# ami-iit/jaxsim

Measured on AMD Instinct MI355X. Metric: env-steps/sec (whole node), iCub 23-DoF soft-contact, batch 1024/8192, higher is better.
Workload: dtype f32

## Files before the change

### include/jaxsim_amd.h

```cpp
#ifndef JAXSIM_AMD_H
#define JAXSIM_AMD_H

#include <stdint.h>

#ifdef __cplusplus
extern "C" {
#endif

#define JXS_OK 0
#define JXS_EINVAL (-1)
#define JXS_ENODEVICE (-2)
#define JXS_ENOMEM (-3)
#define JXS_ECOMM (-4)

#define JXS_F32 0
#define JXS_F64 1

#define JXS_REPR_INERTIAL 0
#define JXS_REPR_BODY 1
#define JXS_REPR_MIXED 2

#define JXS_INTEGRATOR_SEMI_IMPLICIT_EULER 0
#define JXS_INTEGRATOR_RUNGE_KUTTA4 1
#define JXS_INTEGRATOR_RUNGE_KUTTA4_FAST 2
// ... 6 lines not shown
  int32_t n_links;
  int32_t floating_base;
  int32_t dtype;
  const int32_t* parent;
  const int32_t* joint_type;
  const double* joint_axis;
  const double* lambda_H_pre;
  const double* suc_H_i;
  const double* link_mass;
  const double* link_com;
  const double* link_inertia;
  const double* friction_static;
  const double* friction_viscous;
  const double* position_limit_min;
  const double* position_limit_max;
  const double* position_limit_spring;
  const double* position_limit_damper;
  int32_t n_points;
  const int32_t* point_body;
  const double* point_position;
  const uint8_t* point_enabled;
  double time_step;
  double gravity;
  double K, D, mu, p, q;
  double terrain_height;
  double torque_max, omega_th, omega_max;
  int32_t enable_friction;
  double terrain_normal[3];
  int32_t integrator;
  int32_t contact_model;
  double regularization_delassus;
  double solver_tol;
  double rr_time_constant, rr_damping_coefficient, rr_d_min, rr_d_max, rr_width, rr_midpoint, rr_power;
  const double* terrain_grid;
  int32_t terrain_nx, terrain_ny;
  double terrain_origin[2];
  double terrain_spacing[2];
  double terrain_delta;
} jxs_model_desc;

typedef struct jxs_model jxs_model;

typedef struct jxs_layout {
  int32_t n_links, n_joints, n_points, n_rows;
  int32_t row_pos, row_quat, row_s, row_vlin, row_vang, row_sd, row_m;
  int32_t group;
  int32_t tile;
  int32_t dtype;
  int32_t row_mode;
} jxs_layout;

const char* jxs_last_error(void);
int jxs_device_count(int* count);
int jxs_set_device(int device);
int jxs_malloc(void** dptr, uint64_t bytes);
int jxs_free(void* dptr);
int jxs_memcpy_h2d(void* dst, const void* src, uint64_t bytes, void* stream);
int jxs_memcpy_d2h(void* dst, const void* src, uint64_t bytes, void* stream);
int jxs_memcpy_d2d(void* dst, const void* src, uint64_t bytes, void* stream);
int jxs_memset(void* dst, int value, uint64_t bytes, void* stream);
int jxs_stream_create(void** stream);
int jxs_stream_destroy(void* stream);
int jxs_stream_synchronize(void* stream);
int jxs_stream_wait_spin(void* stream);
int jxs_device_synchronize(void);
int jxs_event_create(void** event);
int jxs_event_destroy(void* event);
int jxs_event_record(void* event, void* stream);
int jxs_event_elapsed_ms(void* start, void* stop, float* ms);

int jxs_model_create(const jxs_model_desc* desc, jxs_model** out);
int jxs_model_destroy(jxs_model* model);
int jxs_model_layout(const jxs_model* model, jxs_layout* out);

enum { JXS_MODE_STEP = 0, JXS_MODE_STEP_RIGID = 6 };
int jxs_kernel_spec(const jxs_model_desc* desc, int mode, char* buf, int capacity);
int jxs_model_attach_specialized(jxs_model* model, int mode, const char* shared_object_path);
int jxs_model_specialized_modes(const jxs_model* model, unsigned* mask);


int jxs_step(jxs_model* model, const void* state_in, void* state_out, const void* tau,
             const void* link_forces, int force_repr, int N, void* stream);

int jxs_step_repeat(jxs_model* model, void* state, const void* tau, const void* link_forces,
                    int force_repr, int N, int n_launches, void* stream);

int jxs_step_repeat_timed(jxs_model* model, void* state, const void* tau, const void* link_forces,
                          int force_repr, int N, int n_launches, void* stream, double* seconds);

int jxs_rollout(jxs_model* model, void* state, const void* tau, const void* link_forces,
                int force_repr, int N, int n_steps, void* stream);

int jxs_rollout_controlled(jxs_model* model, void* state, const void* tau_seq, const void* link_forces,
                           int force_repr, int N, int n_steps, void* stream);

int jxs_rollout_recorded(jxs_model* model, void* state, const void* tau, int tau_per_step, const void* link_forces,
                         int force_repr, int N, int n_steps, void* out_states, void* stream);

int jxs_forward_dynamics_aba(jxs_model* model, const void* state, const void* joint_forces,
                             const void* link_forces, int force_repr, void* out_acc, int N,
                             void* stream);

int jxs_system_dynamics(jxs_model* model, const void* state, const void* joint_torques, const void* link_forces,
                        int force_repr, double baumgarte, void* out_xdot, void* out_link_contact_forces, int N,
                        void* stream);
int jxs_link_contact_forces(jxs_model* model, const void* state, const void* joint_torques, const void* link_forces,
                            int force_repr, void* out_link_contact_forces, void* out_mdot, int N, void* stream);

int jxs_inverse_dynamics(jxs_model* model, const void* state, const void* in_acc,
                         const void* link_forces, int force_repr, void* out_forces, int N,
                         void* stream);

int jxs_tile_from_env_major(const void* src, void* dst, int rows, int N, int tile, int dtype, void* stream);
int jxs_tile_to_env_major(const void* src, void* dst, int rows, int N, int tile, int dtype, void* stream);

int jxs_validate_state(jxs_model* model, const void* state, int N, int* counts3, void* stream);

int jxs_env_select(const uint8_t* mask, const void* a, const void* b, void* out, int rows, int N, int tile, int dtype,
                   void* stream);

int jxs_env_copy(const void* src, int src_N, int src_tile, const int32_t* src_idx, void* dst, int dst_N, int dst_tile,
                 const int32_t* dst_idx, int rows, int K, int dtype, void* stream);

enum { JXS_ENV_NONFINITE = 1, JXS_ENV_QUAT_NOT_UNIT = 2 };
int jxs_env_flags(jxs_model* model, const void* state, int N, uint8_t* out_flags, void* stream);

int jxs_env_randomize(jxs_model* model, const uint8_t* mask, void* state, int N, const void* bounds, uint64_t seed,
                      uint64_t draw, int64_t first_env, int velocity_representation, void* stream);

#define JXS_OBS_MAX_WIDTH 4096
enum {
  JXS_OBS_STATE_ROW = 0,
  JXS_OBS_SOURCE_ROW = 1,
  JXS_OBS_BASE_QUAT_UNIT = 2,
  JXS_OBS_BASE_ROTATION = 3,
  JXS_OBS_BASE_VELOCITY = 4,
  JXS_OBS_PROJECTED_GRAVITY = 5
};
typedef struct jxs_observation jxs_observation;
int jxs_observation_create(jxs_model* model, int D, const int32_t* slots , const double* offset,
                           const double* scale, const int32_t source_rows[4], jxs_observation** out);
int jxs_observation_destroy(jxs_observation* observation);
int jxs_env_observe(jxs_model* model, const jxs_observation* observation, const void* state,
                    const void* const sources[4], int N, int velocity_representation, void* out, int out_dtype,
                    int64_t out_ld, void* stream);

#define JXS_ACT_MAX_WIDTH 4096
enum { JXS_ACT_OFF = 0, JXS_ACT_TORQUE = 1, JXS_ACT_POSITION = 2, JXS_ACT_VELOCITY = 3 };
typedef struct jxs_action jxs_action;
int jxs_action_create(jxs_model* model, int A, const int32_t* joints ,
                      const double* params , jxs_action** out);
int jxs_action_destroy(jxs_action* action);
int jxs_env_act(jxs_model* model, const jxs_action* action, const void* state, const void* actions, int act_dtype,
                int64_t act_ld, const void* feed_forward, void* out_tau, int N, void* stream);

#define JXS_EVAL_MAX_SLOTS 1024
#define JXS_EVAL_MAX_TERMS 32
#define JXS_EVAL_MAX_CONDITIONS 32
#define JXS_DONE_TERMINATED 1
#define JXS_DONE_TRUNCATED 2
enum { JXS_EVAL_IDENTITY = 0, JXS_EVAL_ABS = 1, JXS_EVAL_SQUARE = 2, JXS_EVAL_EXCESS = 3 };
enum { JXS_EVAL_OUTER_IDENTITY = 0, JXS_EVAL_OUTER_EXP = 1 };
enum { JXS_EVAL_TERMINATED = 0, JXS_EVAL_TRUNCATED = 1 };
typedef struct jxs_evaluation_desc {
  int32_t D, K, C;
  const int32_t* slots;
  const int32_t* targets;
  const double* offset;
// ... 96 lines not shown
```

### jaxsim_amd/_lib.py

```python

from __future__ import annotations

import ctypes as C
import os
import pathlib

import numpy as np

_HERE = pathlib.Path(__file__).resolve().parent
LIB_PATH = _HERE / "csrc" / "libjaxsim_amd.so"

JXS_F32, JXS_F64 = 0, 1


class JaxsimAmdError(RuntimeError):
    pass


class ModelDesc(C.Structure):

    _fields_ = [
        ("n_links", C.c_int32),
        ("floating_base", C.c_int32),
        ("dtype", C.c_int32),
# ... 159 lines not shown
    d.regularization_delassus = float(getattr(cm, "regularization_delassus", 1e-6))
    d.solver_tol = float(getattr(cm, "solver_tol", 1e-3))
    return d, keep


def model_signature(model, dtype) -> tuple:
    kdp = model.kin_dyn_parameters
    cp, ap = model.contact_params, model.actuation_params
    return (
        id(kdp), np.dtype(dtype).str, model.time_step, model.gravity, model.floating_base(),
        cp.K, cp.D, cp.mu, getattr(cp, "p", 0.5), getattr(cp, "q", 0.5), model.terrain._height, tuple(getattr(model.terrain, "_normal", (0.0, 0.0, 1.0))),
        ap.torque_max, ap.omega_th, ap.omega_max, ap.enable_friction, int(model.integrator),
        type(model.contact_model).__name__, getattr(model.contact_model, "regularization_delassus", None),
        getattr(model.contact_model, "solver_tol", None),
        tuple(getattr(cp, k, None) for k in ("time_constant", "damping_coefficient", "d_min", "d_max", "width", "midpoint", "power")),
        (id(getattr(model.terrain, "_heights", None)), getattr(model.terrain, "_origin", None), getattr(model.terrain, "_spacing", None),
         getattr(model.terrain, "delta", None)) if getattr(model.terrain, "_heights", None) is not None else None,
    )


_lib = None


def _declare(lib):
    vp, cp_ = C.c_void_p, C.c_char_p
    lib.jxs_last_error.restype = cp_
    lib.jxs_last_error.argtypes = []
    sig = {
        "jxs_device_count": [C.POINTER(C.c_int)],
        "jxs_set_device": [C.c_int],
        "jxs_malloc": [C.POINTER(vp), C.c_uint64],
        "jxs_free": [vp],
        "jxs_memcpy_h2d": [vp, vp, C.c_uint64, vp],
        "jxs_memcpy_d2h": [vp, vp, C.c_uint64, vp],
        "jxs_memcpy_d2d": [vp, vp, C.c_uint64, vp],
        "jxs_memset": [vp, C.c_int, C.c_uint64, vp],
        "jxs_stream_create": [C.POINTER(vp)],
        "jxs_stream_destroy": [vp],
        "jxs_stream_synchronize": [vp],
        "jxs_stream_wait_spin": [vp],
        "jxs_device_synchronize": [],
        "jxs_event_create": [C.POINTER(vp)],
        "jxs_event_destroy": [vp],
        "jxs_event_record": [vp, vp],
        "jxs_event_elapsed_ms": [vp, vp, C.POINTER(C.c_float)],
        "jxs_model_create": [C.POINTER(ModelDesc), C.POINTER(vp)],
        "jxs_kernel_spec": [C.POINTER(ModelDesc), C.c_int, C.c_char_p, C.c_int],
        "jxs_model_attach_specialized": [vp, C.c_int, C.c_char_p],
        "jxs_model_specialized_modes": [vp, C.POINTER(C.c_uint)],
        "jxs_model_destroy": [vp],
        "jxs_model_layout": [vp, C.POINTER(Layout)],
        "jxs_step": [vp, vp, vp, vp, vp, C.c_int, C.c_int, vp],
        "jxs_step_gravity_compensated": [vp, vp, vp, vp, vp, C.c_int, C.c_int, vp],
        "jxs_rollout": [vp, vp, vp, vp, C.c_int, C.c_int, C.c_int, vp],
        "jxs_rollout_controlled": [vp, vp, vp, vp, C.c_int, C.c_int, C.c_int, vp],
        "jxs_rollout_recorded": [vp, vp, vp, C.c_int, vp, C.c_int, C.c_int, C.c_int, vp, vp],
        "jxs_forward_dynamics_aba": [vp, vp, vp, vp, C.c_int, vp, C.c_int, vp],
        "jxs_forward_dynamics_crb": [vp, vp, vp, vp, C.c_int, vp, C.c_int, vp],
        "jxs_inverse_dynamics": [vp, vp, vp, vp, C.c_int, vp, C.c_int, vp],
        "jxs_system_dynamics": [vp, vp, vp, vp, C.c_int, C.c_double, vp, vp, C.c_int, vp],
        "jxs_link_contact_forces": [vp, vp, vp, vp, C.c_int, vp, vp, C.c_int, vp],
        "jxs_gravity_torques": [vp, vp, vp, C.c_int, vp],
        "jxs_tile_from_env_major": [vp, vp, C.c_int, C.c_int, C.c_int, C.c_int, vp],
        "jxs_tile_to_env_major": [vp, vp, C.c_int, C.c_int, C.c_int, C.c_int, vp],
        "jxs_validate_state": [vp, vp, C.c_int, C.POINTER(C.c_int), vp],
        "jxs_env_select": [vp, vp, vp, vp, C.c_int, C.c_int, C.c_int, C.c_int, vp],
        "jxs_env_copy": [vp, C.c_int, C.c_int, vp, vp, C.c_int, C.c_int, vp, C.c_int, C.c_int, C.c_int, vp],
        "jxs_env_flags": [vp, vp, C.c_int, vp, vp],
        "jxs_env_randomize": [vp, vp, vp, C.c_int, vp, C.c_uint64, C.c_uint64, C.c_int64, C.c_int, vp],
        "jxs_observation_create": [vp, C.c_int, C.POINTER(C.c_int32), C.POINTER(C.c_double), C.POINTER(C.c_double), C.POINTER(C.c_int32), C.POINTER(vp)],
        "jxs_observation_destroy": [vp],
        "jxs_env_observe": [vp, vp, vp, C.POINTER(vp), C.c_int, C.c_int, vp, C.c_int, C.c_int64, vp],
        "jxs_action_create": [vp, C.c_int, C.POINTER(C.c_int32), C.POINTER(C.c_double), C.POINTER(vp)],
        "jxs_action_destroy": [vp],
        "jxs_env_act": [vp, vp, vp, vp, C.c_int, C.c_int64, vp, vp, C.c_int, vp],
        "jxs_evaluation_create": [vp, C.POINTER(EvaluationDesc), C.POINTER(vp)],
        "jxs_evaluation_destroy": [vp],
        "jxs_env_evaluate": [vp, vp, vp, C.POINTER(vp), C.c_int, C.c_int, vp, C.c_int, vp, vp, vp, C.c_int, C.c_int64, vp, C.c_int, vp],
        "jxs_contact_sensors_create": [vp, C.c_int, C.POINTER(C.c_int32), C.c_int, C.POINTER(C.c_int32), C.POINTER(C.c_double), C.POINTER(vp)],
        "jxs_contact_sensors_destroy": [vp],
        "jxs_env_contacts": [vp, vp, vp, vp, C.c_int, C.c_double, vp, vp, vp, vp],
        "jxs_step_repeat": [vp, vp, vp, vp, C.c_int, C.c_int, C.c_int, vp],
        "jxs_step_repeat_timed": [vp, vp, vp, vp, C.c_int, C.c_int, C.c_int, vp, C.POINTER(C.c_double)],
        "jxs_refresh_kinematics": [vp, vp, vp, vp, C.c_int, vp],
        "jxs_mass_matrix": [vp, vp, vp, C.c_int, vp],
        "jxs_centroidal": [vp, vp, vp, vp, C.c_int, vp],
        "jxs_coriolis": [vp, vp, vp, vp, C.c_int, vp],
        "jxs_frames_create": [vp, C.c_int, C.POINTER(C.c_int32), C.POINTER(C.c_double), C.POINTER(vp)],
        "jxs_frames_destroy": [vp],
        "jxs_frame_kinematics": [vp, vp, vp, C.c_int, C.c_int, vp, vp, C.c_int, vp],
        "jxs_solver_fault_counts": [vp, C.POINTER(C.c_int), C.c_int, vp],
        "jxs_debug_reload_env": [],
        "jxs_jacobian_full": [vp, vp, vp, vp, C.c_int, vp],
        "jxs_mass_matrix_inverse": [vp, vp, vp, C.c_int, vp],
        "jxs_comm_unique_id": [C.c_char * 128],
        "jxs_comm_version": [C.POINTER(C.c_int)],
        "jxs_device_pci_bus_id": [C.c_char_p, C.c_int],
        "jxs_comm_init": [C.POINTER(vp), C.c_char * 128, C.c_int, C.c_int],
        "jxs_comm_destroy": [vp],
        "jxs_allgather": [vp, vp, vp, C.c_uint64, C.c_int, vp],
    }
    for name, args in sig.items():
        fn = getattr(lib, name)
        fn.restype = C.c_int
        fn.argtypes = args
    return sig


EXPORTED_SYMBOLS = None


def load(path: os.PathLike | None = None):
    global _lib, EXPORTED_SYMBOLS
    if _lib is not None and path is None:
        return _lib
    override = os.environ.get("JAXSIM_AMD_LIB")
    p = pathlib.Path(path) if path is not None else (pathlib.Path(override) if override else LIB_PATH)
    if not p.exists():
        raise JaxsimAmdError(
            f"HIP extension not built: {p} is missing. Run `python -c 'import __graft_entry__ as g; g.build()'` "
            "(or jaxsim_amd/csrc/build.sh). There is no CPU fallback."
        )
    try:
        lib = C.CDLL(str(p))
    except OSError as e:
        raise JaxsimAmdError(f"cannot load {p}: {e}") from e
    EXPORTED_SYMBOLS = tuple(_declare(lib).keys()) + ("jxs_last_error",)
    if path is None:
        _lib = lib
    return lib


def check(rc: int, what: str = "") -> None:
    if rc != 0:
        msg = load().jxs_last_error()
        raise JaxsimAmdError(f"{what} failed ({rc}): {msg.decode() if msg else ''}")
```

### jaxsim_amd/csrc/jxs_api.hip

```cpp
#include <cstdint>
#include <dlfcn.h>
#include <hip/hip_runtime.h>

#include <algorithm>
#include <atomic>
#include <chrono>
#include <rccl/rccl.h>

#include <cstdlib>
#include <cstring>
#include <map>
#include <memory>
#include <mutex>
#include <string>
#include <type_traits>

#include "../../include/jaxsim_amd.h"
#include "jxs_env_act.h"
#include "jxs_env_contact.h"
#include "jxs_env_evaluate.h"
#include "jxs_env_observe.h"
#include "jxs_env_ops.h"
#include "jxs_env_random.h"
#include "jxs_params.h"
// ... 887 lines not shown

namespace {

int refuse(const char* who, const std::string& what) { return fail(JXS_EINVAL, std::string(who) + ": " + what); }

bool repr_ok(int r) { return r == JXS_REPR_INERTIAL || r == JXS_REPR_BODY || r == JXS_REPR_MIXED; }

struct EnvTile {
  int tile = 0, tile_shift = 0;
};
int env_tile(const char* who, int G, int rows, EnvTile& t) {
  t.tile = G > 0 ? 64 / G : 0, t.tile_shift = 0;
  while ((1 << t.tile_shift) < t.tile) ++t.tile_shift;
  if (t.tile <= 0 || (1 << t.tile_shift) != t.tile || t.tile > 64) return refuse(who, "the model's tile does not divide the wave");
  if (jxs_env::tile_words(rows, t.tile) >= (1LL << 30)) return refuse(who, "rows * tile must be below 2^30");
  return JXS_OK;
}

template <int WB, typename F>
void with_access(int access, F&& f) {
  if (access == 16) f(std::integral_constant<int, 16>{});
  else if (access == 8) f(std::integral_constant<int, 8>{});
  else if constexpr (WB == 4) f(std::integral_constant<int, 4>{});
}
template <typename T, typename F>
void with_io_type(bool models_own, F&& f) {
  if (models_own) f(T{});
  else f(float{});
}

constexpr int kEnvBlock = 256;
dim3 env_grid(long long waves) { return dim3((unsigned)((waves + 3) / 4)); }
long long env_waves(int N, int env_shift) { return ((long long)N + (1LL << env_shift) - 1) >> env_shift; }

int launched(const char* who) {
  const hipError_t e = hipGetLastError();
  return e != hipSuccess ? hip_fail(e, who) : (int)JXS_OK;
}

template <typename Table, typename KP>
bool table_fits(const Table& t, int dtype, const KP& P) {
  return t.dtype == dtype && t.n_rows == P.n_rows && t.n_joints == P.n;
}

void* upload_table(const std::vector<unsigned char>& host, const char* what) {
  void* d = nullptr;
  hipError_t e = hipMalloc(&d, host.size());
  if (e == hipSuccess && (e = hipMemcpy(d, host.data(), host.size(), hipMemcpyHostToDevice)) != hipSuccess) (void)hipFree(d);
  if (e == hipSuccess) return d;
  hip_fail(e, what);
  return nullptr;
}
template <typename Table>
int destroy_table(Table* t) {
  if (t != nullptr) (void)hipFree(t->table);
  delete t;
  return JXS_OK;
}

template <typename T>
int attach_typed(jxs_model* model, ModelT<T>* mt, int mode, const char* path) {
  const std::string want = jxs::kernel_spec_string(mt->pk, mode);
  void* h = dlopen(path, RTLD_NOW | RTLD_LOCAL);
  if (h == nullptr) return fail(JXS_EINVAL, std::string("cannot load the specialised kernel: ") + dlerror());
  auto text = reinterpret_cast<const char* (*)()>(dlsym(h, "jxs_spec_string"));
  auto launch = reinterpret_cast<typename ModelT<T>::SpecLaunch>(dlsym(h, "jxs_spec_launch"));
  if (text == nullptr || launch == nullptr) {
    dlclose(h);
    return fail(JXS_EINVAL, "not a specialised-kernel object (jxs_spec_string / jxs_spec_launch missing)");
  }
  if (want != text()) {
    const std::string got = text();
    dlclose(h);
    return fail(JXS_EINVAL, "the specialised kernel was built for another model: " + got + " != " + want);
  }
  mt->spec_handle[mode] = h;
  mt->spec_launch[mode] = launch;
  static std::atomic<unsigned long long> next_uid{1ull << 40};
  model->uid = next_uid.fetch_add(1);
  return JXS_OK;
}
}

extern "C" {

int jxs_debug_set_stamp_buffer(void* dptr) {
  g_dbg = static_cast<long long*>(dptr);
  return JXS_OK;
}

const char* jxs_last_error(void) { return g_err.c_str(); }

int jxs_device_count(int* count) {
  if (count == nullptr) return fail(JXS_EINVAL, "null count");
  hipError_t e = hipGetDeviceCount(count);
  if (e != hipSuccess) {
    *count = 0;
    return hip_fail(e, "hipGetDeviceCount");
  }
  return JXS_OK;
}
int jxs_set_device(int device) {
  JXS_HIP(hipSetDevice(device));
  return JXS_OK;
}
int jxs_malloc(void** dptr, uint64_t bytes) {
  if (dptr == nullptr) return fail(JXS_EINVAL, "null dptr");
  hipError_t e = hipMalloc(dptr, bytes > 0 ? bytes : 1);
  if (e == hipErrorOutOfMemory) return fail(JXS_ENOMEM, "hipMalloc: out of memory");
  if (e != hipSuccess) return hip_fail(e, "hipMalloc");
  return JXS_OK;
}
int jxs_free(void* dptr) {
  JXS_HIP(hipFree(dptr));
  return JXS_OK;
}
int jxs_memcpy_h2d(void* dst, const void* src, uint64_t bytes, void* stream) {
  JXS_HIP(hipMemcpyAsync(dst, src, bytes, hipMemcpyHostToDevice, static_cast<hipStream_t>(stream)));
  JXS_HIP(hipStreamSynchronize(static_cast<hipStream_t>(stream)));
  return JXS_OK;
}
int jxs_memcpy_d2h(void* dst, const void* src, uint64_t bytes, void* stream) {
  JXS_HIP(hipMemcpyAsync(dst, src, bytes, hipMemcpyDeviceToHost, static_cast<hipStream_t>(stream)));
  JXS_HIP(hipStreamSynchronize(static_cast<hipStream_t>(stream)));
  return JXS_OK;
}
int jxs_memcpy_d2d(void* dst, const void* src, uint64_t bytes, void* stream) {
  JXS_HIP(hipMemcpyAsync(dst, src, bytes, hipMemcpyDeviceToDevice, static_cast<hipStream_t>(stream)));
  return JXS_OK;
}
int jxs_memset(void* dst, int value, uint64_t bytes, void* stream) {
  JXS_HIP(hipMemsetAsync(dst, value, bytes, static_cast<hipStream_t>(stream)));
  return JXS_OK;
}
int jxs_stream_create(void** stream) {
  if (stream == nullptr) return fail(JXS_EINVAL, "null stream");
  hipStream_t s;
  JXS_HIP(hipStreamCreateWithFlags(&s, hipStreamNonBlocking));
  *stream = s;
  return JXS_OK;
}
int jxs_stream_destroy(void* stream) {
  JXS_HIP(hipStreamDestroy(static_cast<hipStream_t>(stream)));
  return JXS_OK;
}
int jxs_stream_synchronize(void* stream) {
  JXS_HIP(hipStreamSynchronize(static_cast<hipStream_t>(stream)));
  return JXS_OK;
}
int jxs_stream_wait_spin(void* stream) {
  hipStream_t s = static_cast<hipStream_t>(stream);
  for (;;) {
    const hipError_t e = hipStreamQuery(s);
    if (e == hipSuccess) return JXS_OK;
    if (e != hipErrorNotReady) return hip_fail(e, "hipStreamQuery");
  }
}
int jxs_device_synchronize(void) {
  JXS_HIP(hipDeviceSynchronize());
  return JXS_OK;
}
int jxs_event_create(void** event) {
  if (event == nullptr) return fail(JXS_EINVAL, "null event");
  hipEvent_t e;
  JXS_HIP(hipEventCreate(&e));
  *event = e;
// ... 574 lines not shown
int jxs_env_contacts(jxs_model* model, const jxs_contact_sensors* sensors, const void* link_transforms, const void* link_velocities, int N, double dt,
                     const uint8_t* reset_mask, void* timers, void* out_record, void* stream) {
  const char* const who = "jxs_env_contacts";
  if (model == nullptr || sensors == nullptr || link_transforms == nullptr || out_record == nullptr) return refuse(who, "null argument");
  if (N <= 0) return refuse(who, "N must be positive");
  const jxs_contact_sensors& cs = *sensors;
  hipStream_t s = static_cast<hipStream_t>(stream);
  return with_typed(model, [&](auto* mt) {
    using T = typename std::remove_pointer_t<decltype(mt)>::value_type;
    const auto& KP = mt->pk.P;
    if (!(dt >= 0.0) || !jxs_obs::affine_ok(dt, T(0))) return refuse(who, "dt must be finite in the model's dtype and not negative");
    if (!table_fits(cs, model->dtype, KP) || cs.n_links != KP.nL) return refuse(who, "the contact-sensor table was created for another model layout or dtype");
    EnvTile t;
    if (const int rc = env_tile(who, mt->pk.G, std::max(12 * KP.nL, jxs_contact::kRows * cs.G), t)) return rc;
    if ((uintptr_t)link_transforms % sizeof(T) != 0 || (uintptr_t)link_velocities % sizeof(T) != 0 || (uintptr_t)timers % sizeof(T) != 0 ||
        (uintptr_t)out_record % sizeof(T) != 0)
      return refuse(who, "link_transforms, link_velocities, timers and out_record must be aligned to their element type");
    const int want = knob(g_contact_envs_per_wave);
    const int env_shift = jxs_env::env_shift_for(N, t.tile_shift, want > 0 ? want : t.tile);
    const int chunk = std::max(1, std::min(cs.P, 512 >> env_shift));
    const size_t per_wave = (size_t)((2 * chunk + 3 * cs.G) << env_shift) * sizeof(T);
    int waves_per_block = 4;
    while (waves_per_block > 1 && waves_per_block * per_wave > 64 * 1024) waves_per_block >>= 1;
    const unsigned char* b = static_cast<const unsigned char*>(cs.table);
    const ContactTable<T> tb{reinterpret_cast<const int32_t*>(b), reinterpret_cast<const int32_t*>(b + cs.parent_at), reinterpret_cast<const T*>(b + cs.points_at),
                             cs.G, cs.P};
    jxs_contact::Terrain<T> tr{};
    tr.kind = KP.hf ? jxs_contact::kTerrainField : KP.flat ? jxs_contact::kTerrainFlat : jxs_contact::kTerrainPlane;
    tr.height = KP.terrain_h;
    for (int k = 0; k < 3; ++k) tr.normal[k] = KP.nrm[k];
    tr.inv_nz = T(1) / KP.nrm[2];
    tr.nx = KP.hf_nx, tr.ny = KP.hf_ny, tr.x0 = KP.hf_x0, tr.y0 = KP.hf_y0, tr.idx = KP.hf_idx, tr.idy = KP.hf_idy;
    tr.delta = KP.hf_delta, tr.inv_2delta = KP.hf_inv_2delta;
    tr.samples = reinterpret_cast<const T*>(mt->mblk + KP.hf_off);
    const dim3 grid = env_grid(env_waves(N, env_shift) * (4 / waves_per_block));
    hipLaunchKernelGGL((jxs_env_contacts_kernel<T>), grid, dim3(64 * waves_per_block), waves_per_block * per_wave, s, static_cast<const T*>(link_transforms),
                       static_cast<const T*>(link_velocities), tb, tr, KP.nL, N, t.tile_shift, env_shift, chunk, static_cast<T>(dt), reset_mask,
                       static_cast<T*>(timers), static_cast<T*>(out_record));
    return launched(who);
  });
}

int jxs_step(jxs_model* model, const void* state_in, void* state_out, const void* tau, const void* link_forces,
             int force_repr, int N, void* stream) {
  if (state_out == nullptr) return fail(JXS_EINVAL, "null state_out");
  return run(model, step_request(state_in, state_out, tau, link_forces, force_repr, N, 1), stream);
}
int jxs_step_gravity_compensated(jxs_model* model, const void* state_in, void* state_out, const void* tau,
                                 const void* link_forces, int force_repr, int N, void* stream) {
  if (state_out == nullptr) return fail(JXS_EINVAL, "null state_out");
  if (model == nullptr) return fail(JXS_EINVAL, "null model");
  if (!with_typed(model, [](auto* mt) { return mt->pk.P.rigid != 0; }))
    return fail(JXS_EINVAL, "jxs_step_gravity_compensated: built for the rigid contact models (RigidContacts / RelaxedRigidContacts with "
                            "enabled points); use jxs_gravity_torques + jxs_step");
  Launch L = step_request(state_in, state_out, tau, link_forces, force_repr, N, 1);
  L.flags = kFlagGravityCompensated;
  return run(model, L, stream);
}
int jxs_rollout(jxs_model* model, void* state, const void* tau, const void* link_forces, int force_repr, int N,
                int n_steps, void* stream) {
  if (n_steps < 0) return fail(JXS_EINVAL, "n_steps must be >= 0");
  return run(model, step_request(state, state, tau, link_forces, force_repr, N, n_steps), stream);
}
int jxs_rollout_controlled(jxs_model* model, void* state, const void* tau_seq, const void* link_forces, int force_repr,
                           int N, int n_steps, void* stream) {
  if (n_steps < 0) return fail(JXS_EINVAL, "n_steps must be >= 0");
  if (n_steps == 0) return JXS_OK;
  if (tau_seq == nullptr) return fail(JXS_EINVAL, "null torque sequence (jxs_rollout takes constant or no torques)");
  Launch L = step_request(state, state, tau_seq, link_forces, force_repr, N, n_steps);
  if (n_steps > 1) L.flags = kFlagTauSequence;
  return run(model, L, stream);
}
int jxs_rollout_recorded(jxs_model* model, void* state, const void* tau, int tau_per_step, const void* link_forces,
                         int force_repr, int N, int n_steps, void* out_states, void* stream) {
  if (n_steps < 0) return fail(JXS_EINVAL, "n_steps must be >= 0");
  if (n_steps == 0) return JXS_OK;
  if (out_states == nullptr) return fail(JXS_EINVAL, "null out_states (jxs_rollout / jxs_rollout_controlled do not record)");
  if (tau_per_step && tau == nullptr) return fail(JXS_EINVAL, "tau_per_step without a torque sequence");
  Launch L = step_request(state, state, tau, link_forces, force_repr, N, n_steps);
  if (tau_per_step && n_steps > 1) L.flags = kFlagTauSequence;
  L.traj = out_states;
  return run(model, L, stream);
}
int jxs_step_repeat(jxs_model* model, void* state, const void* tau, const void* link_forces, int force_repr, int N,
                    int n_launches, void* stream) {
  if (n_launches < 0) return fail(JXS_EINVAL, "n_launches must be >= 0");
  if (n_launches == 0) return JXS_OK;
  if (model == nullptr) return fail(JXS_EINVAL, "null model");
  if (state == nullptr) return fail(JXS_EINVAL, "null state");
  Launch L = step_request(state, state, tau, link_forces, force_repr, N, n_launches);
  L.fuse = false;
  static const bool use_graph = std::getenv("JXS_DISABLE_STEP_GRAPH") == nullptr;
  static const int kShort = std::getenv("JXS_STEP_GRAPH_LAUNCHES") ? std::max(2, std::atoi(std::getenv("JXS_STEP_GRAPH_LAUNCHES"))) : 50;
  static const int kLong = std::max(kShort, 250);
  if (use_graph && stream != nullptr && n_launches >= 2) {
    struct Key {
      unsigned long long m; void* st; const void* tau; const void* lf; int repr, N; void* s; int block;
      bool operator==(const Key& o) const {
        return m == o.m && st == o.st && tau == o.tau && lf == o.lf && repr == o.repr && N == o.N && s == o.s && block == o.block;
      }
    };
    struct Slot {
      Key key{};
      hipGraphExec_t exec = nullptr;
    };
    static const bool graph_remainder = std::getenv("JXS_STEP_GRAPH_REMAINDER") != nullptr;
    static thread_local Slot slots[3];
    hipStream_t hs = static_cast<hipStream_t>(stream);
    for (int t = (kLong > kShort ? 0 : 1); t < (graph_remainder ? 3 : 2); ++t) {
      const int block = t == 0 ? kLong : t == 1 ? kShort : n_launches;
      if (block < 2 || n_launches < block) continue;
      const Key k{model->uid, state, tau, link_forces, force_repr, N, stream, block};
      Slot& sl = slots[t];
      if (sl.exec == nullptr || !(k == sl.key)) {
        if (sl.exec != nullptr) (void)hipGraphExecDestroy(sl.exec), sl.exec = nullptr;
        hipGraph_t g = nullptr;
        JXS_HIP(hipStreamBeginCapture(hs, hipStreamCaptureModeThreadLocal));
        L.repeat = block;
        const int rc = run(model, L, stream);
        hipError_t e = hipStreamEndCapture(hs, &g);
        if (rc != JXS_OK) {
          if (g != nullptr) (void)hipGraphDestroy(g);
          return rc;
        }
        if (e != hipSuccess) return hip_fail(e, "hipStreamEndCapture");
        e = hipGraphInstantiate(&sl.exec, g, nullptr, nullptr, 0);
        (void)hipGraphDestroy(g);
        if (e != hipSuccess) {
          sl.exec = nullptr;
          return hip_fail(e, "hipGraphInstantiate");
        }
        sl.key = k;
      }
      for (; n_launches >= block; n_launches -= block) JXS_HIP(hipGraphLaunch(sl.exec, hs));
    }
    if (n_launches == 0) return JXS_OK;
  }
  L.repeat = n_launches;
  return run(model, L, stream);
}
int jxs_step_repeat_timed(jxs_model* model, void* state, const void* tau, const void* link_forces, int force_repr, int N,
                          int n_launches, void* stream, double* seconds) {
  if (seconds == nullptr) return fail(JXS_EINVAL, "null seconds");
  int rc = jxs_stream_wait_spin(stream);
  if (rc != JXS_OK) return rc;
  const auto t0 = std::chrono::steady_clock::now();
  rc = jxs_step_repeat(model, state, tau, link_forces, force_repr, N, n_launches, stream);
  if (rc != JXS_OK) return rc;
  static const bool by_query = std::getenv("JXS_TIMED_WAIT_QUERY") != nullptr;
  static volatile uint32_t* line = [] {
    void* p = nullptr;
    if (hipHostMalloc(&p, 64 * sizeof(uint32_t), hipHostMallocDefault) != hipSuccess) return static_cast<volatile uint32_t*>(nullptr);
    std::memset(p, 0, 64 * sizeof(uint32_t));
    return static_cast<volatile uint32_t*>(p);
  }();
  static std::atomic<int> next_word{0};
  static thread_local int my_word = -1;
  static thread_local uint32_t seq = 0;
  if (my_word < 0) my_word = next_word.fetch_add(1);
  volatile uint32_t* flag = (line != nullptr && my_word < 64) ? line + my_word : nullptr;
  bool polled = false;
  if (!by_query && flag != nullptr && stream != nullptr) {
    const uint32_t want = ++seq;
    hipStream_t hs = static_cast<hipStream_t>(stream);
    if (hipStreamWriteValue32(hs, const_cast<uint32_t*>(flag), want, 0) == hipSuccess) {
      polled = true;
      for (unsigned spins = 0; *flag != want; ++spins) {
        if ((spins & 4095u) == 4095u) {
          const hipError_t q = hipStreamQuery(hs);
          if (q == hipSuccess) break;
          if (q != hipErrorNotReady) return hip_fail(q, "hipStreamQuery");
        }
      }
      const hipError_t q = hipStreamQuery(hs);
      if (q != hipSuccess && q != hipErrorNotReady) return hip_fail(q, "hipStreamQuery");
    } else {
      (void)hipGetLastError();
    }
  }
  if (!polled) rc = jxs_stream_wait_spin(stream);
  *seconds = std::chrono::duration<double>(std::chrono::steady_clock::now() - t0).count();
  return rc;
}
static int forward_dynamics(jxs_model* model, int mode, const void* state, const void* joint_forces, const void* link_forces,
                            int force_repr, void* out_acc, int N, void* stream) {
  if (out_acc == nullptr) return fail(JXS_EINVAL, "null out_acc");
  Launch L = request(mode, state, N, joint_forces, link_forces, force_repr);
  L.out_a = out_acc;
  return run(model, L, stream);
}
int jxs_forward_dynamics_aba(jxs_model* model, const void* state, const void* joint_forces, const void* link_forces,
                             int force_repr, void* out_acc, int N, void* stream) {
  return forward_dynamics(model, jxs::MODE_FD, state, joint_forces, link_forces, force_repr, out_acc, N, stream);
}
int jxs_forward_dynamics_crb(jxs_model* model, const void* state, const void* joint_forces, const void* link_forces,
                             int force_repr, void* out_acc, int N, void* stream) {
  return forward_dynamics(model, jxs::MODE_FD_CRB, state, joint_forces, link_forces, force_repr, out_acc, N, stream);
}
static int run_dynamics(jxs_model* model, const void* state, const void* joint_torques, const void* link_forces, int force_repr,
                        double baumgarte, void* out_xdot, void* out_link_contact_forces, int N, void* stream) {
  Launch L = request(jxs::MODE_DYN, state, N, joint_torques, link_forces, force_repr);
  L.state_out = out_xdot;
  L.out_H = out_link_contact_forces;
  L.fparam = baumgarte;
  return run(model, L, stream);
}
int jxs_system_dynamics(jxs_model* model, const void* state, const void* joint_torques, const void* link_forces,
                        int force_repr, double baumgarte, void* out_xdot, void* out_link_contact_forces, int N, void* stream) {
  if (out_xdot == nullptr && out_link_contact_forces == nullptr) return fail(JXS_EINVAL, "jxs_system_dynamics: no output asked for");
  if (out_xdot != nullptr && out_xdot == state) return fail(JXS_EINVAL, "jxs_system_dynamics: out_xdot must not alias the state");
  return run_dynamics(model, state, joint_torques, link_forces, force_repr, baumgarte, out_xdot, out_link_contact_forces, N, stream);
}
int jxs_link_contact_forces(jxs_model* model, const void* state, const void* joint_torques, const void* link_forces,
                            int force_repr, void* out_link_contact_forces, void* out_mdot, int N, void* stream) {
  if (out_link_contact_forces == nullptr) return fail(JXS_EINVAL, "null out_link_contact_forces");
  if (model == nullptr) return fail(JXS_EINVAL, "null model");
  if (N <= 0) return fail(JXS_EINVAL, "N must be positive");
  jxs_layout lay;
  jxs_model_layout(model, &lay);
  if (out_mdot == nullptr || lay.n_points == 0)
    return run_dynamics(model, state, joint_torques, link_forces, force_repr, 1.0, nullptr, out_link_contact_forces, N, stream);
  const size_t tile_bytes = (size_t)lay.tile * (model->dtype == JXS_F64 ? 8 : 4);
  hipStream_t s = static_cast<hipStream_t>(stream);
// ... 211 lines not shown
```

Measured before the change: 161.5 million.

## Split step_repeat batch into concurrent chains on forked streams

When the batch needs more waves than the device can keep resident and there are enough repeated launches, step_repeat now splits the environments into up to two (at most four) contiguous chunks. Each chunk runs its own repeat loop and cached graph on a separate non-blocking stream, forked from and joined back to the caller's stream. The aim is to let the tail of one chunk's launch overlap with the start of the next, reducing idle CUs at kernel boundaries. In exchange it adds per-chain streams, events and graph slots, and chunks may compete for the device or fall slightly out of balance.

Measured after the change: 161.5 million. About the same (-0.0%).

```diff
diff --git a/include/jaxsim_amd.h b/include/jaxsim_amd.h
--- a/include/jaxsim_amd.h
+++ b/include/jaxsim_amd.h
@@ -112,8 +112,13 @@
 int jxs_step(jxs_model* model, const void* state_in, void* state_out, const void* tau,
              const void* link_forces, int force_repr, int N, void* stream);
 
+#define JXS_STEP_MAX_CHAINS 4
 int jxs_step_repeat(jxs_model* model, void* state, const void* tau, const void* link_forces,
                     int force_repr, int N, int n_launches, void* stream);
+
+int jxs_step_chain_plan(jxs_model* model, int N, int n_launches, int max_chains, int* bounds, int* n_chains);
+int jxs_step_chain_plan_resident(int N, int T, long long resident_waves, int n_launches, int max_chains,
+                                 int* bounds, int* n_chains);
 
 int jxs_step_repeat_timed(jxs_model* model, void* state, const void* tau, const void* link_forces,
                           int force_repr, int N, int n_launches, void* stream, double* seconds);
diff --git a/jaxsim_amd/_lib.py b/jaxsim_amd/_lib.py
--- a/jaxsim_amd/_lib.py
+++ b/jaxsim_amd/_lib.py
@@ -265,6 +265,8 @@
         "jxs_env_contacts": [vp, vp, vp, vp, C.c_int, C.c_double, vp, vp, vp, vp],
         "jxs_step_repeat": [vp, vp, vp, vp, C.c_int, C.c_int, C.c_int, vp],
         "jxs_step_repeat_timed": [vp, vp, vp, vp, C.c_int, C.c_int, C.c_int, vp, C.POINTER(C.c_double)],
+        "jxs_step_chain_plan": [vp, C.c_int, C.c_int, C.c_int, C.POINTER(C.c_int), C.POINTER(C.c_int)],
+        "jxs_step_chain_plan_resident": [C.c_int, C.c_int, C.c_longlong, C.c_int, C.c_int, C.POINTER(C.c_int), C.POINTER(C.c_int)],
         "jxs_refresh_kinematics": [vp, vp, vp, vp, C.c_int, vp],
         "jxs_mass_matrix": [vp, vp, vp, C.c_int, vp],
         "jxs_centroidal": [vp, vp, vp, vp, C.c_int, vp],
diff --git a/jaxsim_amd/csrc/jxs_api.hip b/jaxsim_amd/csrc/jxs_api.hip
--- a/jaxsim_amd/csrc/jxs_api.hip
+++ b/jaxsim_amd/csrc/jxs_api.hip
@@ -993,6 +993,84 @@
 }
 }
 
+namespace {
+
+constexpr int kMaxChains = JXS_STEP_MAX_CHAINS;
+constexpr int kShortGraphBlock = 50;
+
+int split_chains(int N, int T, int chains, int* bounds) {
+  const long long tiles = ((long long)N + T - 1) / T, groups = (tiles + 3) / 4;
+  const int n = (int)std::max(1ll, std::min<long long>({(long long)chains, (long long)kMaxChains, groups}));
+  for (int c = 0; c < n; ++c) bounds[c] = (int)(groups * c / n * 4 * T);
+  bounds[n] = N;
+  return n;
+}
+constexpr int kAutoChains = 2;
+int auto_chains(int N, int T, long long resident_waves, int n_launches, int max_chains) {
+  const long long waves = ((long long)N + T - 1) / T;
+  if (waves <= resident_waves || n_launches < kShortGraphBlock) return 1;
+  return std::max(1, std::min({kAutoChains, max_chains, kMaxChains}));
+}
+
+template <typename T>
+int step_waves_per_cu(const ModelT<T>* mt) {
+  const auto& P = mt->pk.P;
+  if (P.rigid || mt->pk.integrator == JXS_INTEGRATOR_RUNGE_KUTTA4 || P.n_chunks > 1) return 0;
+  const size_t lds = P.row_mode ? sizeof(T) * (size_t)(64 / mt->pk.G) * jxs::lds_rows_words(mt->pk.G, P.nL) : 0;
+  const int by_regs = 3 * 4;
+  return lds == 0 ? by_regs : (int)std::min<size_t>(by_regs, (size_t)160 * 1024 / lds);
+}
+long long step_resident_waves(const jxs_model* model) {
+  static std::atomic<int> cus_of[64] = {};
+  int dev = 0, cus = 0;
+  if (hipGetDevice(&dev) != hipSuccess || dev < 0 || dev >= 64) return (void)hipGetLastError(), 0;
+  if ((cus = cus_of[dev].load(std::memory_order_relaxed)) == 0) {
+    if (hipDeviceGetAttribute(&cus, hipDeviceAttributeMultiprocessorCount, dev) != hipSuccess || cus <= 0) return (void)hipGetLastError(), 0;
+    cus_of[dev].store(cus, std::memory_order_relaxed);
+  }
+  return (long long)cus * with_typed(model, [](auto* mt) { return step_waves_per_cu(mt); });
+}
+
+struct ChainStreams {
+  hipStream_t stream[kMaxChains] = {};
+  hipEvent_t joined[kMaxChains] = {};
+  hipEvent_t fork = nullptr;
+  int n = 0;
+  bool grow(int want) {
+    if (fork == nullptr && hipEventCreateWithFlags(&fork, hipEventDisableTiming) != hipSuccess) return fork = nullptr, (void)hipGetLastError(), false;
+    for (; n < want; ++n) {
+      if (hipStreamCreateWithFlags(&stream[n], hipStreamNonBlocking) != hipSuccess) return stream[n] = nullptr, (void)hipGetLastError(), false;
+      if (hipEventCreateWithFlags(&joined[n], hipEventDisableTiming) != hipSuccess) {
+        (void)hipGetLastError();
+        (void)hipStreamDestroy(stream[n]);
+        return stream[n] = nullptr, joined[n] = nullptr, false;
+      }
+    }
+    return true;
+  }
+};
+ChainStreams* chain_streams(int want) {
+  static thread_local ChainStreams per_device[64];
+  int dev = 0;
+  if (hipGetDevice(&dev) != hipSuccess || dev < 0 || dev >= 64) return (void)hipGetLastError(), nullptr;
+  return per_device[dev].grow(want) ? &per_device[dev] : nullptr;
+}
+
+struct StepGraphKey {
+  unsigned long long m; void* st; const void* tau; const void* lf; int repr, N, first; void* s; int block;
+  bool operator==(const StepGraphKey& o) const {
+    return m == o.m && st == o.st && tau == o.tau && lf == o.lf && repr == o.repr && N == o.N && first == o.first && s == o.s && block == o.block;
+  }
+};
+struct StepGraphSlot {
+  StepGraphKey key{};
+  hipGraphExec_t exec = nullptr;
+};
+
+int step_repeat_chain(jxs_model* model, Launch L, int first_env, int n_launches, void* stream, StepGraphSlot* slots);
+
+}
+
 extern "C" {
 
 int jxs_debug_set_stamp_buffer(void* dptr) {
@@ -1733,6 +1811,32 @@
   L.traj = out_states;
   return run(model, L, stream);
 }
+int jxs_step_chain_plan_resident(int N, int T, long long resident_waves, int n_launches, int max_chains, int* bounds, int* n_chains) {
+  if (bounds == nullptr || n_chains == nullptr) return fail(JXS_EINVAL, "null bounds or n_chains");
+  if (N <= 0 || n_launches < 0 || max_chains < 1) return fail(JXS_EINVAL, "N and max_chains must be positive, n_launches not negative");
+  if (T < 1 || T > 64 || (T & (T - 1)) != 0) return fail(JXS_EINVAL, "T = 64 / G, a power of two in [1, 64]");
+  *n_chains = split_chains(N, T, auto_chains(N, T, resident_waves, n_launches, max_chains), bounds);
+  return JXS_OK;
+}
+static int plan_chains(const jxs_model* model, int N, int n_launches, int max_chains, int* bounds) {
+  const char* const chains_env = std::getenv("JXS_STEP_CHAINS");
+  const int forced = chains_env == nullptr ? 0 : std::atoi(chains_env);
+  const int T = 64 / with_typed(model, [](auto* mt) { return mt->pk.G; });
+  bounds[0] = 0, bounds[1] = N;
+  if (forced >= 2) return split_chains(N, T, std::min(forced, max_chains), bounds);
+  if (forced == 1 || n_launches < kShortGraphBlock || N <= 4 * T) return 1;
+  const long long resident = step_resident_waves(model);
+  if (resident <= 0) return 1;
+  return split_chains(N, T, auto_chains(N, T, resident, n_launches, max_chains), bounds);
+}
+int jxs_step_chain_plan(jxs_model* model, int N, int n_launches, int max_chains, int* bounds, int* n_chains) {
+  if (model == nullptr) return fail(JXS_EINVAL, "null model");
+  if (bounds == nullptr || n_chains == nullptr) return fail(JXS_EINVAL, "null bounds or n_chains");
+  if (N <= 0 || n_launches < 0 || max_chains < 1) return fail(JXS_EINVAL, "N and max_chains must be positive, n_launches not negative");
+  *n_chains = plan_chains(model, N, n_launches, max_chains, bounds);
+  return JXS_OK;
+}
+
 int jxs_step_repeat(jxs_model* model, void* state, const void* tau, const void* link_forces, int force_repr, int N,
                     int n_launches, void* stream) {
   if (n_launches < 0) return fail(JXS_EINVAL, "n_launches must be >= 0");
@@ -1741,28 +1845,64 @@
   if (state == nullptr) return fail(JXS_EINVAL, "null state");
   Launch L = step_request(state, state, tau, link_forces, force_repr, N, n_launches);
   L.fuse = false;
+  static thread_local StepGraphSlot slots[1 + kMaxChains][3];
+  int bounds[kMaxChains + 1] = {0, N}, n_chains = 1;
+  hipStream_t hs = static_cast<hipStream_t>(stream);
+  if (stream != nullptr && N > 0 && (n_chains = plan_chains(model, N, n_launches, kMaxChains, bounds)) > 1) {
+    hipStreamCaptureStatus capturing = hipStreamCaptureStatusNone;
+    if (hipStreamIsCapturing(hs, &capturing) != hipSuccess) (void)hipGetLastError(), capturing = hipStreamCaptureStatusActive;
+    if (capturing != hipStreamCaptureStatusNone) n_chains = 1;
+  }
+  ChainStreams* const cs = n_chains > 1 ? chain_streams(n_chains) : nullptr;
+  if (cs == nullptr) return step_repeat_chain(model, L, 0, n_launches, stream, slots[0]);
+  if (force_repr < 0 || force_repr > 2) return fail(JXS_EINVAL, "invalid force representation");
+  JXS_HIP(hipEventRecord(cs->fork, hs));
+  for (int c = 0; c < n_chains; ++c) JXS_HIP(hipStreamWaitEvent(cs->stream[c], cs->fork, 0));
+  int rc = JXS_OK;
+  std::string err;
+  with_typed(model, [&](auto* mt) {
+    using T = typename std::remove_pointer_t<decltype(mt)>::value_type;
+    const auto& P = mt->pk.P;
+    const size_t tile_bytes = sizeof(T) * (size_t)(64 / mt->pk.G);
+    for (int c = 0; c < n_chains && rc == JXS_OK; ++c) {
+      const size_t tile0 = (size_t)bounds[c] / (64 / mt->pk.G);
+      auto at = [&](const void* p, size_t rows) { return p == nullptr ? nullptr : static_cast<const char*>(p) + tile0 * rows * tile_bytes; };
+      Launch Lc = L;
+      Lc.N = bounds[c + 1] - bounds[c];
+      Lc.state_in = at(state, P.n_rows);
+      Lc.state_out = const_cast<char*>(at(state, P.n_rows));
+      Lc.tau = at(tau, P.n);
+      Lc.link_f = at(link_forces, (size_t)P.nL * 6);
+      rc = step_repeat_chain(model, Lc, bounds[c], n_launches, cs->stream[c], slots[1 + c]);
+      if (rc != JXS_OK) err = g_err;
+    }
+    return 0;
+  });
+  for (int c = 0; c < n_chains; ++c) {
+    hipError_t e = hipEventRecord(cs->joined[c], cs->stream[c]);
+    if (e == hipSuccess) e = hipStreamWaitEvent(hs, cs->joined[c], 0);
+    if (e != hipSuccess && rc == JXS_OK) rc = hip_fail(e, "joining the step chains"), err = g_err;
+  }
+  if (rc != JXS_OK) g_err = err;
+  return rc;
+}
+
+namespace {
+int step_repeat_chain(jxs_model* model, Launch L, int first_env, int n_launches, void* stream, StepGraphSlot* slots) {
+  const void* const state = L.state_in;
+  const void *const tau = L.tau, *const link_forces = L.link_f;
+  const int force_repr = L.force_repr, N = L.N;
   static const bool use_graph = std::getenv("JXS_DISABLE_STEP_GRAPH") == nullptr;
   static const int kShort = std::getenv("JXS_STEP_GRAPH_LAUNCHES") ? std::max(2, std::atoi(std::getenv("JXS_STEP_GRAPH_LAUNCHES"))) : 50;
   static const int kLong = std::max(kShort, 250);
   if (use_graph && stream != nullptr && n_launches >= 2) {
-    struct Key {
-      unsigned long long m; void* st; const void* tau; const void* lf; int repr, N; void* s; int block;
-      bool operator==(const Key& o) const {
-        return m == o.m && st == o.st && tau == o.tau && lf == o.lf && repr == o.repr && N == o.N && s == o.s && block == o.block;
-      }
-    };
-    struct Slot {
-      Key key{};
-      hipGraphExec_t exec = nullptr;
-    };
     static const bool graph_remainder = std::getenv("JXS_STEP_GRAPH_REMAINDER") != nullptr;
-    static thread_local Slot slots[3];
     hipStream_t hs = static_cast<hipStream_t>(stream);
     for (int t = (kLong > kShort ? 0 : 1); t < (graph_remainder ? 3 : 2); ++t) {
       const int block = t == 0 ? kLong : t == 1 ? kShort : n_launches;
       if (block < 2 || n_launches < block) continue;
-      const Key k{model->uid, state, tau, link_forces, force_repr, N, stream, block};
-      Slot& sl = slots[t];
+      const StepGraphKey k{model->uid, const_cast<void*>(state), tau, link_forces, force_repr, N, first_env, stream, block};
+      StepGraphSlot& sl = slots[t];
       if (sl.exec == nullptr || !(k == sl.key)) {
         if (sl.exec != nullptr) (void)hipGraphExecDestroy(sl.exec), sl.exec = nullptr;
         hipGraph_t g = nullptr;
@@ -1790,6 +1930,8 @@
   L.repeat = n_launches;
   return run(model, L, stream);
 }
+}
+
 int jxs_step_repeat_timed(jxs_model* model, void* state, const void* tau, const void* link_forces, int force_repr, int N,
                           int n_launches, void* stream, double* seconds) {
   if (seconds == nullptr) return fail(JXS_EINVAL, "null seconds");
```
